# baegwangbin/MaGNet

Hardware: NVIDIA B200
Metric: frames/sec (640x480, 4 views, 64 hyp) (higher is better)
Workload: dtype f32

## Files before the change

### magnet_b200/csrc/cost_mma.cu

```cuda
#include <cuda_fp16.h>

#include <algorithm>
#include <atomic>
#include <cstddef>
#include <mutex>
#include <type_traits>

#include "common.cuh"
#include "tma_common.cuh"

namespace magnet {

constexpr int MNT = 256;
constexpr int MTW = 8, MTH = 8;
constexpr int MPX = MTW * MTH;
constexpr int MCH = 64;
constexpr int MSEG = 32;
constexpr int MMAXV = 16;
constexpr int M_TMEM_COLS = 256;
constexpr int SEG_BYTES = 2048;
constexpr int META_SEG_BYTES = 128;

constexpr int MOFF_A = 0;
constexpr int MOFF_R = 16384;
constexpr int MR_BYTES = 67584;
constexpr int MOFF_META = MOFF_R + MR_BYTES;
constexpr int MOFF_CAM = MOFF_META + MSEG * META_SEG_BYTES;
constexpr int MOFF_KS = MOFF_CAM + MMAXV * 64;
constexpr int MOFF_BBOX = MOFF_KS + MCH * 4;
constexpr int MOFF_BAR = MOFF_BBOX + 64;
constexpr int MOFF_ACC = MOFF_BAR + 64;
constexpr int MOFF_PIX = MOFF_ACC + MCH * 65 * 4;
constexpr int M_SMEM_USED = MOFF_PIX + 8 * 8 * 32;
constexpr int M_SMEM_TOTAL = M_SMEM_USED + 1024;
static_assert(MR_BYTES >= MSEG * SEG_BYTES && MR_BYTES >= MPX * 260 * 4 && MR_BYTES >= MCH * 65 * 4, "region R");
static_assert(2 * (M_SMEM_TOTAL + 1024) <= 227 * 1024, "two CTAs per SM");

struct Split16Header {
  float scale;
  float inv_scale;
  unsigned absmax;
};
constexpr size_t SPLIT16_HEADER = 256;

__host__ __device__ inline size_t split16_bytes(size_t N, size_t H, size_t W) {
  return SPLIT16_HEADER + N * H * W * 256 + N * H * (W + 1) * 16;
}

__device__ __forceinline__ void mbar_wait_or_trap(uint32_t bar, uint32_t parity) {
#pragma unroll 1
  for (int it = 0; it < (1 << 22); ++it) {
    uint32_t done;
    asm volatile("{\n.reg .pred P1;\nmbarrier.try_wait.parity.shared::cta.b64 P1, [%1], %2, %3;\nselp.u32 %0, 1, 0, P1;\n}"
                 : "=r"(done) : "r"(bar), "r"(parity), "r"(20000u) : "memory");
    if (done) return;
  }
  __trap();
}

constexpr int MMA_SLOTS = 1024;
__device__ unsigned g_mma_next[MMA_SLOTS];
__device__ unsigned g_mma_done[MMA_SLOTS];

__device__ __forceinline__ float lds_f32(uint32_t a) {
  float v;
  asm volatile("ld.shared.f32 %0, [%1];" : "=f"(v) : "r"(a));
  return v;
}
__device__ __forceinline__ float4 lds_f32x4(uint32_t a) {
  float4 v;
  asm volatile("ld.shared.v4.f32 {%0, %1, %2, %3}, [%4];" : "=f"(v.x), "=f"(v.y), "=f"(v.z), "=f"(v.w) : "r"(a));
  return v;
}
__device__ __forceinline__ float2 lerp2d_x2(float4 top, float4 bot, float fx, float fy) {
  const float2 v00 = make_float2(top.x, top.y), v01 = make_float2(top.z, top.w);
  const float2 v10 = make_float2(bot.x, bot.y), v11 = make_float2(bot.z, bot.w);
  const float2 m1 = make_float2(-1.0f, -1.0f), fx2 = make_float2(fx, fx), fy2 = make_float2(fy, fy);
  const float2 t = __ffma2_rn(fx2, __ffma2_rn(v00, m1, v01), v00), u = __ffma2_rn(fx2, __ffma2_rn(v10, m1, v11), v10);
  return __ffma2_rn(fy2, __ffma2_rn(t, m1, u), t);
}

template <int MODE, bool CW>
__global__ void __launch_bounds__(MNT, 2)
cost_mma_kernel(const __grid_constant__ CostParams p, const __grid_constant__ CUtensorMap tm_ref,
                const __grid_constant__ CUtensorMap tm_src, const __grid_constant__ CUtensorMap tm_meta, const int nchunks,
                const int n_items, const int slot, float* __restrict__ dbg) {
  extern __shared__ unsigned char smem_raw[];
  const uint32_t raw = smem_u32(smem_raw);
  const uint32_t padb = (1024u - (raw & 1023u)) & 1023u;
  unsigned char* smem = smem_raw + padb;
  const uint32_t sbase = raw + padb;
  const magnet_camera* cams_s = reinterpret_cast<const magnet_camera*>(smem + MOFF_CAM);
  float* ks = reinterpret_cast<float*>(smem + MOFF_KS);
  int* bbox = reinterpret_cast<int*>(smem + MOFF_BBOX);
  float* regR = reinterpret_cast<float*>(smem + MOFF_R);
  const uint32_t bar_tma = sbase + MOFF_BAR, bar_mma = sbase + MOFF_BAR + 8, bar_cam = sbase + MOFF_BAR + 24;
  float* acc_s = reinterpret_cast<float*>(smem + MOFF_ACC);
  const unsigned FULL = 0xffffffffu;

  const int tid = threadIdx.x, lane = tid & 31, warp = tid >> 5;
  const int H = p.H, W = p.W, HW = p.HW, D = p.D, V = p.V;
  const int tiles_x = (W + MTW - 1) / MTW;
  const int items_per_b = tiles_x * ((H + MTH - 1) / MTH) * nchunks;

  const unsigned char* refbuf = reinterpret_cast<const unsigned char*>(p.ref_feat);
  const unsigned char* srcbuf = reinterpret_cast<const unsigned char*>(p.src_feat);
  const Split16Header* hdr_ref = reinterpret_cast<const Split16Header*>(refbuf);
  const Split16Header* hdr_src = reinterpret_cast<const Split16Header*>(srcbuf);
  volatile int* next_item = reinterpret_cast<volatile int*>(smem + MOFF_BAR + 40);

  if (tid == 0) {
    mbar_init(bar_tma, 1);
    mbar_init(bar_mma, 1);
    mbar_init(bar_cam, 1);
    fence_mbar_init();
    prefetch_tmap(&tm_ref);
    prefetch_tmap(&tm_src);
    prefetch_tmap(&tm_meta);
  }
  if (warp == 1) tmem_alloc(sbase + MOFF_BAR + 32, M_TMEM_COLS);
  if (tid < 8) bbox[tid] = (tid & 1) ? -(1 << 28) : (1 << 28);
  tmem_fence_before_sync();
  __syncthreads();
  tmem_fence_after_sync();
  const uint32_t tmem_base = *reinterpret_cast<const volatile uint32_t*>(smem + MOFF_BAR + 32);
  uint32_t ph_tma = 0, ph_mma = 0, ph_cam = 0;
  int it = 0;
  int cur_b = -1;
  const float xmax = (float)W + 1.0f, ymax = (float)H + 1.0f;
  const float kappa = p.kappa;
  const uint32_t g_row0 = sbase + MOFF_R, m_base = sbase + MOFF_META;

  int item = blockIdx.x;
  while (item < n_items) {
  const int b = item / items_per_b;
  const int rem = item - b * items_per_b;
  const int tile = rem / nchunks;
  const int jc = (rem - tile * nchunks) * MCH;
  const int Dc = min(MCH, D - jc);
  const int tx0 = (tile % tiles_x) * MTW, ty0 = (tile / tiles_x) * MTH;

  if (tid == 0) {
    if (b != cur_b) {
      mbar_arrive_expect_tx(bar_cam, (uint32_t)V * 64u);
      bulk_load(sbase + MOFF_CAM, p.cams + (size_t)b * V, (uint32_t)V * 64u, bar_cam);
    }
    tma_load_5d(sbase + MOFF_A, &tm_ref, bar_tma, 0, tx0, ty0, 0, b);
    *next_item = (int)gridDim.x + (int)atomicAdd(&g_mma_next[slot], 1u);
  }
  if (tid < MCH) ks[tid] = MODE != MAGNET_DEPTH_VOLUME ? p.k[min(jc + tid, D - 1)] : 0.0f;
  for (int idx = tid; idx < MCH * 65; idx += MNT) acc_s[idx] = 0.0f;
  __syncthreads();

  const int py = ty0 + warp;
  float R0, R1, R2, MU = 0.f, SG = 0.f;
  unsigned livemask;
  {
    const int px = tx0 + (lane & 7);
    const bool live = px < W && py < H;
    const int n = min(py, H - 1) * W + min(px, W - 1);
    R0 = ldg_f(p.rays + ((size_t)b * 3 + 0) * HW + n);
    R1 = ldg_f(p.rays + ((size_t)b * 3 + 1) * HW + n);
    R2 = ldg_f(p.rays + ((size_t)b * 3 + 2) * HW + n);
    if (MODE == MAGNET_DEPTH_GAUSS) {
      MU = ldg_f(p.ref_gmm + ((size_t)b * 2 + 0) * HW + n);
      SG = ldg_f(p.ref_gmm + ((size_t)b * 2 + 1) * HW + n);
    }
    livemask = __ballot_sync(FULL, live) & 0xffu;
  }
  float2 dvol[MODE == MAGNET_DEPTH_VOLUME ? MTW : 1];
  float2 k2 = make_float2(0.f, 0.f);
  if (MODE == MAGNET_DEPTH_VOLUME) {
    for (int idx = tid; idx < MCH * MPX; idx += MNT) {
      const int j = idx >> 6, pp = idx & 63;
      const int y = ty0 + (pp >> 3), x = tx0 + (pp & 7);
      const size_t n = (size_t)min(y, H - 1) * W + min(x, W - 1);
      regR[j * 65 + pp] = ldg_f(p.d_volume + ((size_t)b * D + jc + min(j, Dc - 1)) * HW + n);
    }
    __syncthreads();
#pragma unroll
    for (int i = 0; i < MTW; ++i) dvol[i] = make_float2(regR[lane * 65 + warp * 8 + i], regR[(lane + 32) * 65 + warp * 8 + i]);
    fence_proxy_async();
    __syncthreads();
  } else {
    k2 = make_float2(ks[lane], ks[lane + 32]);
  }
  auto depth2 = [&](const int i, const float mu, const float sg) -> float2 {
    if (MODE == MAGNET_DEPTH_VOLUME) return dvol[i];
    if (MODE == MAGNET_DEPTH_PLANES) return k2;
    return __fadd2_rn(make_float2(mu, mu), make_float2(__fmul_rn(sg, k2.x), __fmul_rn(sg, k2.y)));
  };
  float4* pixt = reinterpret_cast<float4*>(smem + MOFF_PIX) + warp * 16;

  if (b != cur_b) {
    mbar_wait_or_trap(bar_cam, ph_cam);
    ph_cam ^= 1u;
    cur_b = b;
  }
  bool first = true;

  for (int v = 0; v < V; ++v) {
    const magnet_camera* cam = cams_s + v;
    if (cam->valid != 1.0f) continue;
    const float a0 = cam->a[0], a1 = cam->a[1], a2 = cam->a[2];
    const float Q0 = __fmaf_rn(cam->A[2], R2, __fmaf_rn(cam->A[1], R1, __fmul_rn(cam->A[0], R0)));
    const float Q1 = __fmaf_rn(cam->A[5], R2, __fmaf_rn(cam->A[4], R1, __fmul_rn(cam->A[3], R0)));
    const float Q2 = __fmaf_rn(cam->A[8], R2, __fmaf_rn(cam->A[7], R1, __fmul_rn(cam->A[6], R0)));
    __syncwarp();
    if (lane < 8) {
      pixt[2 * lane] = make_float4(Q0, Q1, Q2, 0.0f);
      pixt[2 * lane + 1] = make_float4(Q2, MU, SG, 0.0f);
    }
    __syncwarp();
    const int vb = v * p.B + b;

    float2 cix[MTW], ciy[MTW];
    float xl = 1e9f, xh = -1e9f, yl = 1e9f, yh = -1e9f;
#pragma unroll
    for (int i = 0; i < MTW; ++i) {
      const float4 t1 = pixt[2 * i], t2 = pixt[2 * i + 1];
      float2 ix, iy, z;
      project2(depth2(i, t2.y, t2.z), a0, a1, a2, t1.x, t1.y, t1.z, ix, iy, z);
      ix.x = fminf(fmaxf(ix.x, -2.0f), xmax); ix.y = fminf(fmaxf(ix.y, -2.0f), xmax);
      iy.x = fminf(fmaxf(iy.x, -2.0f), ymax); iy.y = fminf(fmaxf(iy.y, -2.0f), ymax);
      cix[i] = ix;
      ciy[i] = iy;
      if ((livemask >> i) & 1u) {
        xl = fminf(xl, fminf(ix.x, ix.y)); xh = fmaxf(xh, fmaxf(ix.x, ix.y));
        yl = fminf(yl, fminf(iy.x, iy.y)); yh = fmaxf(yh, fmaxf(iy.x, iy.y));
      }
    }
    int* bb = bbox + (it & 1) * 4;
    {
      const int r0 = __reduce_min_sync(FULL, (int)floorf(xl)), r1 = __reduce_max_sync(FULL, (int)floorf(xh));
      const int r2 = __reduce_min_sync(FULL, (int)floorf(yl)), r3 = __reduce_max_sync(FULL, (int)floorf(yh));
      if (lane == 0) { atomicMin(bb + 0, r0); atomicMax(bb + 1, r1); atomicMin(bb + 2, r2); atomicMax(bb + 3, r3); }
    }
    fence_proxy_async();
    __syncthreads();
    const int wx0 = bb[0], wx1 = bb[1], wy0 = bb[2], wy1 = bb[3];
    if (tid < 4) bbox[((it + 1) & 1) * 4 + tid] = (tid & 1) ? -(1 << 28) : (1 << 28);
    ++it;
    const int nseg_all = (wx1 - wx0 + 2 + 7) >> 3, rows_all = wy1 - wy0 + 2;
    const int nsw = min(nseg_all, 16);
    const int rmax = nseg_all * rows_all <= MSEG ? rows_all : max(2, MSEG / nsw);
    const int stepx = 8 * nsw - 1, stepy = rmax - 1;

    for (int sy = wy0; sy <= wy1; sy += stepy) {
      const int rows = min(stepy, wy1 - sy + 1) + 1;
      for (int sx = wx0; sx <= wx1; sx += stepx) {
        const int nseg = (min(stepx, wx1 - sx + 1) + 1 + 7) >> 3;
        const int nsegs = nseg * rows;
        if (tid == 0)
          mbar_arrive_expect_tx(bar_tma, (uint32_t)nsegs * (SEG_BYTES + (CW ? META_SEG_BYTES : 0)) + (first ? 16384u : 0u));
        first = false;
        if (lane == 0) {
          for (int s = warp; s < nsegs; s += MNT / 32) {
            const int r = s / nseg, xb = s - r * nseg;
            tma_load_5d(sbase + MOFF_R + (uint32_t)s * SEG_BYTES, &tm_src, bar_tma, 0, sx + 8 * xb, sy + r, 0, vb);
            if (CW) tma_load_4d(m_base + (uint32_t)s * META_SEG_BYTES, &tm_meta, bar_tma, 0, sx + 8 * xb + 1, sy + r, vb);
          }
        }
        __syncwarp();
        const int npad = (nsegs * 8 + 15) & ~15;
        const int gp = (((npad + 27) >> 5) << 5) + 4;
        mbar_wait_or_trap(bar_tma, ph_tma);
        ph_tma ^= 1u;
        if (warp == 0) {
          tmem_fence_after_sync();
          if (lane == 0) {
            const uint32_t idesc = umma_idesc_f16(128, (uint32_t)npad);
            const uint64_t a_hi = umma_desc_sw128(sbase + MOFF_A, 1024), a_lo = umma_desc_sw128(sbase + MOFF_A + 8192, 1024);
            const uint64_t b_hi = umma_desc_sw128(sbase + MOFF_R, SEG_BYTES), b_lo = umma_desc_sw128(sbase + MOFF_R + 1024, SEG_BYTES);
            uint32_t accum = 0;
#pragma unroll
            for (int pr = 0; pr < 3; ++pr) {
              const uint64_t ad = pr == 0 ? a_lo : a_hi, bd = pr == 1 ? b_lo : b_hi;
#pragma unroll
              for (int kk = 0; kk < 4; ++kk) {
                umma_f16(tmem_base, ad + 2u * kk, bd + 2u * kk, idesc, accum);
                accum = 1;
              }
            }
            umma_commit(bar_mma);
          }
          __syncwarp();
        }
        mbar_wait_or_trap(bar_mma, ph_mma);
        ph_mma ^= 1u;
        tmem_fence_after_sync();
        if ((warp & 3) < 2) {
          const int row = (warp & 3) * 32 + lane;
          float4* grow = reinterpret_cast<float4*>(regR + (size_t)row * gp);
          for (int cc = warp >> 2; cc * 16 < npad; cc += 2) {
            float t[16];
            tmem_ld16(tmem_base + ((uint32_t)((warp & 3) * 32) << 16) + (uint32_t)(cc * 16), t);
#pragma unroll
            for (int e = 0; e < 4; ++e) grow[cc * 4 + e] = make_float4(t[4 * e], t[4 * e + 1], t[4 * e + 2], t[4 * e + 3]);
          }
        }
        tmem_fence_before_sync();
        __syncthreads();
#ifdef MAGNET_MMA_DEBUG
        if (dbg != nullptr && item == 0 && v == 0 && sy == wy0 && sx == wx0) {
          if (tid == 0) {
            dbg[0] = (float)sx; dbg[1] = (float)sy; dbg[2] = (float)nseg; dbg[3] = (float)rows; dbg[4] = (float)npad;
            dbg[5] = (float)gp; dbg[6] = (float)v; dbg[7] = 3.0f; dbg[8] = hdr_ref->scale; dbg[9] = hdr_src->scale;
          }
          for (int idx = tid; idx < MPX * npad; idx += MNT) dbg[16 + (idx / npad) * 256 + idx % npad] = regR[(idx / npad) * gp + idx % npad];
        }
#endif
        const bool single = nseg_all * rows_all <= MSEG;
        auto phase_c = [&](auto single_tag) {
          constexpr bool SINGLE = decltype(single_tag)::value;
          const float MAGIC = 12582912.0f;
          const float sxf = (float)sx, syf = (float)sy;
          const float xend = sx + stepx > wx1 ? 1e9f : (float)(sx + stepx), yend = sy + stepy > wy1 ? 1e9f : (float)(sy + stepy);
          const float pitch4f = (float)(nseg * 32);
          const float c0f = MAGIC - 4.0f * sxf - pitch4f * syf;
          const uint32_t pitch4 = (uint32_t)nseg * 32u;
          uint32_t rowaddr = g_row0 + (uint32_t)(warp * 8 * gp) * 4u;
          float* accp = acc_s + lane * 65 + warp * 8;
#pragma unroll
          for (int i = 0; i < MTW; ++i, rowaddr += (uint32_t)gp * 4u) {
            if (!((livemask >> i) & 1u)) continue;
            asm volatile("" : "+f"(cix[i].x), "+f"(cix[i].y), "+f"(ciy[i].x), "+f"(ciy[i].y));
            const float2 x = cix[i], y = ciy[i];
            const float2 x0 = make_float2(floorf(x.x), floorf(x.y)), y0 = make_float2(floorf(y.x), floorf(y.y));
            const float2 m1 = make_float2(-1.0f, -1.0f);
            const float2 fx = __ffma2_rn(x0, m1, x), fy = __ffma2_rn(y0, m1, y);
            const float2 o = __ffma2_rn(y0, make_float2(pitch4f, pitch4f), __ffma2_rn(x0, make_float2(4.0f, 4.0f), make_float2(c0f, c0f)));
            uint32_t ca = __float_as_uint(o.x) & 0x3fffffu, cb = __float_as_uint(o.y) & 0x3fffffu;
            bool pa = true, pb = true;
            if (!SINGLE) {
              pa = x0.x >= sxf && x0.x < xend && y0.x >= syf && y0.x < yend;
              pb = x0.y >= sxf && x0.y < xend && y0.y >= syf && y0.y < yend;
              ca = pa ? ca : 0u;
              cb = pb ? cb : 0u;
            }
            const uint32_t ga = rowaddr + ca, gb = rowaddr + cb;
            const float2 g00 = make_float2(lds_f32(ga), lds_f32(gb)), g01 = make_float2(lds_f32(ga + 4), lds_f32(gb + 4));
            const float2 g10 = make_float2(lds_f32(ga + pitch4), lds_f32(gb + pitch4));
            const float2 g11 = make_float2(lds_f32(ga + pitch4 + 4), lds_f32(gb + pitch4 + 4));
            const float2 ct = __ffma2_rn(fx, __ffma2_rn(g00, m1, g01), g00), cu = __ffma2_rn(fx, __ffma2_rn(g10, m1, g11), g10);
            const float2 cost = __ffma2_rn(fy, __ffma2_rn(ct, m1, cu), ct);
            const float costa = cost.x, costb = cost.y;
            bool oka, okb;
            if (CW) {
              const uint32_t ma = m_base + ca * 4u, mb = m_base + cb * 4u;
              const float2 msa = lerp2d_x2(lds_f32x4(ma), lds_f32x4(ma + pitch4 * 4u), fx.x, fy.x);
              const float2 msb = lerp2d_x2(lds_f32x4(mb), lds_f32x4(mb + pitch4 * 4u), fx.y, fy.y);
              const float4 t2 = pixt[2 * i + 1];
              const float2 dd = depth2(i, t2.y, t2.z);
              const float2 z = __fadd2_rn(make_float2(a2, a2), make_float2(__fmul_rn(t2.x, dd.x), __fmul_rn(t2.x, dd.y)));
              oka = fabsf(__fsub_rn(z.x, msa.x)) < __fmul_rn(msa.y, kappa);
              okb = fabsf(__fsub_rn(z.y, msb.x)) < __fmul_rn(msb.y, kappa);
            } else {
              oka = fabsf(costa) < 3.0e38f;
              okb = fabsf(costb) < 3.0e38f;
            }
            if (pa && oka) accp[i] += costa;
            if (pb && okb) accp[32 * 65 + i] += costb;
          }
        };
        if (single) phase_c(std::true_type{});
        else phase_c(std::false_type{});
        fence_proxy_async();
        tmem_fence_before_sync();
        __syncthreads();
      }
    }
  }

  if (first) {
    if (tid == 0) mbar_arrive_expect_tx(bar_tma, 16384u);
    mbar_wait_or_trap(bar_tma, ph_tma);
    ph_tma ^= 1u;
  }

  {
    const float inv = hdr_ref->inv_scale * hdr_src->inv_scale;
    const bool exact = p.inv_v_exact != 0.0f;
    auto fin = [&](float a) { a *= inv; return exact ? a * p.inv_v_exact : __fdiv_rn(a, p.vf); };
    if ((W & 3) == 0 && (reinterpret_cast<uintptr_t>(p.out) & 15) == 0) {
      for (int idx = tid; idx < MCH * 16; idx += MNT) {
        const int j = idx >> 4, r = (idx >> 1) & 7, hx = (idx & 1) * 4;
        const int y = ty0 + r, x = tx0 + hx;
        if (j < Dc && x < W && y < H) {
          const float* a = acc_s + j * 65 + r * 8 + hx;
          *reinterpret_cast<float4*>(p.out + ((size_t)b * D + jc + j) * HW + (size_t)y * W + x) =
              make_float4(fin(a[0]), fin(a[1]), fin(a[2]), fin(a[3]));
        }
      }
    } else {
      for (int idx = tid; idx < MCH * MPX; idx += MNT) {
        const int j = idx >> 6, pp = idx & 63;
        const int y = ty0 + (pp >> 3), x = tx0 + (pp & 7);
        if (j < Dc && x < W && y < H) p.out[((size_t)b * D + jc + j) * HW + (size_t)y * W + x] = fin(acc_s[j * 65 + pp]);
      }
    }
  }
  const int nxt = *next_item;
  __syncthreads();
  item = nxt;
  }

  if (tid == 0) {
    __threadfence();
    if (atomicAdd(&g_mma_done[slot], 1u) == gridDim.x - 1) {
      g_mma_next[slot] = 0u;
      g_mma_done[slot] = 0u;
      __threadfence();
    }
  }
  tmem_fence_before_sync();
  __syncthreads();
  if (warp == 1) tmem_dealloc(tmem_base, M_TMEM_COLS);
}

__device__ __forceinline__ unsigned finite_abs_bits(float x) {
  const unsigned u = __float_as_uint(x) & 0x7fffffffu;
  return u >= 0x7f800000u ? 0u : u;
}

__global__ void __launch_bounds__(256) absmax_kernel(const float4* __restrict__ x, size_t n4, const float* __restrict__ tail,
                                                     int ntail, unsigned* __restrict__ out) {
  unsigned m = 0u;
  for (size_t i = (size_t)blockIdx.x * blockDim.x + threadIdx.x; i < n4; i += (size_t)gridDim.x * blockDim.x) {
    const float4 v = __ldg(x + i);
    m = max(max(m, finite_abs_bits(v.x)), finite_abs_bits(v.y));
    m = max(max(m, finite_abs_bits(v.z)), finite_abs_bits(v.w));
  }
  if (blockIdx.x == 0 && (int)threadIdx.x < ntail) m = max(m, finite_abs_bits(tail[threadIdx.x]));
  m = __reduce_max_sync(0xffffffffu, m);
  if ((threadIdx.x & 31) == 0 && m != 0u) atomicMax(out, m);
}

__device__ __forceinline__ int split16_shift(unsigned absmax_bits) {
  const int e = (int)(absmax_bits >> 23) & 0xff;
  if (e == 0 || e == 255) return 0;
  return max(-100, min(100, 14 - (e - 127)));
}

template <int SPX, bool VEC>
__global__ void __launch_bounds__(256) split16_repack_kernel(const float* __restrict__ src, const float* __restrict__ gmm,
                                                             unsigned char* __restrict__ dst, int N, int HW, int W) {
  constexpr int C = 64;
  __shared__ float t[SPX * (C + 1)];
  Split16Header* hdr = reinterpret_cast<Split16Header*>(dst);
  const int sh = split16_shift(hdr->absmax);
  const float s = __uint_as_float((unsigned)(127 + sh) << 23);
  if (blockIdx.x == 0 && blockIdx.y == 0 && threadIdx.x == 0) {
    hdr->scale = s;
    hdr->inv_scale = __uint_as_float((unsigned)(127 - sh) << 23);
  }
  const size_t img = blockIdx.y;
  const int p0 = blockIdx.x * SPX;
  if constexpr (VEC) {
    static_assert(SPX == 128, "thread mapping below");
    constexpr int CPI = 8;
    const int lane = threadIdx.x & 31, warp = threadIdx.x >> 5;
    const int q4 = (warp & 3) * 8 + (lane & 7), c0 = (warp >> 2) * 4 + (lane >> 3);
    float4 v[C / CPI];
#pragma unroll
    for (int e = 0; e < C / CPI; ++e) {
      const int c = c0 + e * CPI, pix = p0 + 4 * q4;
      v[e] = pix < HW ? __ldg(reinterpret_cast<const float4*>(src + (img * C + c) * HW + pix)) : make_float4(0.f, 0.f, 0.f, 0.f);
    }
#pragma unroll
    for (int e = 0; e < C / CPI; ++e) {
      const int c = c0 + e * CPI;
      t[(4 * q4 + 0) * (C + 1) + c] = v[e].x;
      t[(4 * q4 + 1) * (C + 1) + c] = v[e].y;
      t[(4 * q4 + 2) * (C + 1) + c] = v[e].z;
      t[(4 * q4 + 3) * (C + 1) + c] = v[e].w;
    }
  } else {
    const int xi = threadIdx.x % SPX, cy = threadIdx.x / SPX;
    for (int c = cy; c < C; c += 256 / SPX) t[xi * (C + 1) + c] = p0 + xi < HW ? src[(img * C + c) * HW + p0 + xi] : 0.0f;
  }
  __syncthreads();
  __half* planes = reinterpret_cast<__half*>(dst + SPLIT16_HEADER);
  float4* meta = reinterpret_cast<float4*>(dst + SPLIT16_HEADER + (size_t)N * HW * 256);
#pragma unroll
  for (int itw = 0; itw < SPX * 8 / 256; ++itw) {
    const int item = itw * 256 + threadIdx.x;
    const int pl = item >> 3, q = item & 7;
    if (p0 + pl < HW) {
      __align__(16) __half hi[8], lo[8];
#pragma unroll
      for (int e = 0; e < 8; ++e) {
        const float v = t[pl * (C + 1) + q * 8 + e] * s;
        hi[e] = __float2half_rn(v);
        lo[e] = __float2half_rn(v - __half2float(hi[e]));
      }
      const size_t o = (size_t)(p0 + pl) * 64 + q * 8;
      *reinterpret_cast<uint4*>(planes + (img * 2 + 0) * (size_t)HW * 64 + o) = *reinterpret_cast<const uint4*>(hi);
      *reinterpret_cast<uint4*>(planes + (img * 2 + 1) * (size_t)HW * 64 + o) = *reinterpret_cast<const uint4*>(lo);
    }
  }
  if (threadIdx.x < SPX && p0 + threadIdx.x < HW) {
    const int pix = p0 + threadIdx.x;
    const int y = pix / W, x = pix - y * W;
    float2 ms = make_float2(0.0f, 0.0f);
    if (gmm != nullptr) ms = make_float2(gmm[(img * 2 + 0) * HW + pix], gmm[(img * 2 + 1) * HW + pix]);
    float2* row = reinterpret_cast<float2*>(meta + (img * (HW / W) + y) * (size_t)(W + 1));
    row[2 * (x + 1)] = ms;
    row[2 * x + 1] = ms;
    if (x == 0) row[0] = make_float2(0.0f, 0.0f);
    if (x == W - 1) row[2 * W + 1] = make_float2(0.0f, 0.0f);
  }
}

cudaError_t launch_repack_split16(const float* src, const float* gmm, void* dst, int N, int C, int H, int W,
                                  cudaStream_t st, int* launches) {
  if (C != 64) return cudaErrorInvalidValue;
  const int HW = H * W;
  const size_t n = (size_t)N * C * HW;
  cudaError_t e = cudaMemsetAsync(dst, 0, SPLIT16_HEADER, st);
  if (e != cudaSuccess) return e;
  const size_t n4 = n / 4;
  const int blocks = (int)std::min<size_t>(148 * 8, (n4 + 255) / 256 + 1);
  absmax_kernel<<<blocks, 256, 0, st>>>(reinterpret_cast<const float4*>(src), n4, src + n4 * 4, (int)(n - n4 * 4),
                                        reinterpret_cast<unsigned*>(static_cast<unsigned char*>(dst) + offsetof(Split16Header, absmax)));
  dim3 block(256);
  if (HW % 4 == 0 && reinterpret_cast<uintptr_t>(src) % 16 == 0) {
    dim3 grid((HW + 127) / 128, N);
    split16_repack_kernel<128, true><<<grid, block, 0, st>>>(src, gmm, static_cast<unsigned char*>(dst), N, HW, W);
  } else {
    dim3 grid((HW + 31) / 32, N);
    split16_repack_kernel<32, false><<<grid, block, 0, st>>>(src, gmm, static_cast<unsigned char*>(dst), N, HW, W);
  }
  *launches = 2;
  return cudaGetLastError();
}

typedef CUresult (*EncodeTiledFn)(CUtensorMap*, CUtensorMapDataType, cuuint32_t, void*, const cuuint64_t*,
                                  const cuuint64_t*, const cuuint32_t*, const cuuint32_t*, CUtensorMapInterleave,
                                  CUtensorMapSwizzle, CUtensorMapL2promotion, CUtensorMapFloatOOBfill);
EncodeTiledFn encode_tiled_fn();

static cudaError_t make_planes_map(CUtensorMap* tm, const void* planes, int N, int H, int W, int box_rows) {
  EncodeTiledFn enc = encode_tiled_fn();
  if (!enc) return cudaErrorNotSupported;
  const cuuint64_t dims[5] = {64, (cuuint64_t)W, (cuuint64_t)H, 2, (cuuint64_t)N};
  const cuuint64_t strides[4] = {128, (cuuint64_t)W * 128, (cuuint64_t)H * W * 128, (cuuint64_t)H * W * 256};
  const cuuint32_t box[5] = {64u, 8u, (cuuint32_t)box_rows, 2u, 1u};
  const cuuint32_t estr[5] = {1u, 1u, 1u, 1u, 1u};
  const CUresult r = enc(tm, CU_TENSOR_MAP_DATA_TYPE_FLOAT16, 5, const_cast<void*>(planes), dims, strides, box, estr,
                         CU_TENSOR_MAP_INTERLEAVE_NONE, CU_TENSOR_MAP_SWIZZLE_128B, CU_TENSOR_MAP_L2_PROMOTION_L2_256B,
                         CU_TENSOR_MAP_FLOAT_OOB_FILL_NONE);
  return r == CUDA_SUCCESS ? cudaSuccess : cudaErrorInvalidValue;
}

static cudaError_t make_meta_map(CUtensorMap* tm, const void* meta, int N, int H, int W) {
  EncodeTiledFn enc = encode_tiled_fn();
  if (!enc) return cudaErrorNotSupported;
  const cuuint64_t dims[4] = {4, (cuuint64_t)W + 1, (cuuint64_t)H, (cuuint64_t)N};
  const cuuint64_t strides[3] = {16, ((cuuint64_t)W + 1) * 16, (cuuint64_t)H * (W + 1) * 16};
  const cuuint32_t box[4] = {4u, 8u, 1u, 1u};
  const cuuint32_t estr[4] = {1u, 1u, 1u, 1u};
  const CUresult r = enc(tm, CU_TENSOR_MAP_DATA_TYPE_FLOAT32, 4, const_cast<void*>(meta), dims, strides, box, estr,
                         CU_TENSOR_MAP_INTERLEAVE_NONE, CU_TENSOR_MAP_SWIZZLE_NONE, CU_TENSOR_MAP_L2_PROMOTION_L2_128B,
                         CU_TENSOR_MAP_FLOAT_OOB_FILL_NONE);
  return r == CUDA_SUCCESS ? cudaSuccess : cudaErrorInvalidValue;
}

#ifdef MAGNET_MMA_DEBUG
static float* g_mma_dbg = nullptr;
void mma_set_debug_buffer(float* p) { g_mma_dbg = p; }
#endif

static int sm_count(int dev) {
  static int cached[64] = {0};
  int& c = cached[dev & 63];
  if (c == 0) {
    int n = 0;
    if (cudaDeviceGetAttribute(&n, cudaDevAttrMultiProcessorCount, dev) != cudaSuccess || n <= 0) n = 148;
    c = n;
  }
  return c;
}

template <int MODE, bool CW>
static cudaError_t launch_mma_mw(const CostParams& p, cudaStream_t st) {
  static std::once_flag flags[64];
  auto kern = cost_mma_kernel<MODE, CW>;
  int dev = 0;
  cudaError_t e = cudaGetDevice(&dev);
  if (e != cudaSuccess) return e;
  cudaError_t res = cudaSuccess;
  std::call_once(flags[dev & 63], [&] {
    res = cudaFuncSetAttribute(kern, cudaFuncAttributeMaxDynamicSharedMemorySize, M_SMEM_TOTAL);
    if (res == cudaSuccess)
      res = cudaFuncSetAttribute(kern, cudaFuncAttributePreferredSharedMemoryCarveout, cudaSharedmemCarveoutMaxShared);
  });
  if (res != cudaSuccess) return res;
  const int N = p.B * p.V;
  const unsigned char* refbuf = reinterpret_cast<const unsigned char*>(p.ref_feat);
  const unsigned char* srcbuf = reinterpret_cast<const unsigned char*>(p.src_feat);
  CUtensorMap tm_ref, tm_src, tm_meta;
  if ((e = make_planes_map(&tm_ref, refbuf + SPLIT16_HEADER, p.B, p.H, p.W, 8)) != cudaSuccess) return e;
  if ((e = make_planes_map(&tm_src, srcbuf + SPLIT16_HEADER, N, p.H, p.W, 1)) != cudaSuccess) return e;
  if ((e = make_meta_map(&tm_meta, srcbuf + SPLIT16_HEADER + (size_t)N * p.HW * 256, N, p.H, p.W)) != cudaSuccess) return e;
  const int nchunks = (p.D + MCH - 1) / MCH;
  const int tiles = ((p.W + MTW - 1) / MTW) * ((p.H + MTH - 1) / MTH);
  const int n_items = tiles * nchunks * p.B;
  static std::atomic<unsigned> ticket{0}, graph_ticket{0};
  cudaStreamCaptureStatus cap = cudaStreamCaptureStatusNone;
  if (cudaStreamIsCapturing(st, &cap) != cudaSuccess) cap = cudaStreamCaptureStatusNone;
  const int slot = cap == cudaStreamCaptureStatusActive ? MMA_SLOTS / 2 + (int)(graph_ticket.fetch_add(1) % (MMA_SLOTS / 2))
                                                        : (int)(ticket.fetch_add(1) % (MMA_SLOTS / 2));
  dim3 grid(std::min(n_items, 2 * sm_count(dev))), block(MNT);
  float* dbg = nullptr;
#ifdef MAGNET_MMA_DEBUG
  dbg = g_mma_dbg;
#endif
  kern<<<grid, block, M_SMEM_TOTAL, st>>>(p, tm_ref, tm_src, tm_meta, nchunks, n_items, slot, dbg);
  return cudaGetLastError();
}

bool mma_supports(int C, int D, int V, int layout) {
  return C == 64 && layout == MAGNET_SRC_SPLIT16 && D >= 1 && V <= MMAXV;
}

void mma_launch_info(int B, int H, int W, int D, int* grid, int* block, int* smem) {
  int dev = 0;
  cudaGetDevice(&dev);
  *grid = std::min(((W + MTW - 1) / MTW) * ((H + MTH - 1) / MTH) * ((D + MCH - 1) / MCH) * B, 2 * sm_count(dev));
  *block = MNT;
  *smem = M_SMEM_TOTAL;
}

size_t split16_buffer_bytes(int N, int H, int W) { return split16_bytes((size_t)N, (size_t)H, (size_t)W); }

cudaError_t launch_cost_mma(const CostParams& p, int mode, bool cw, cudaStream_t st) {
  if (cw) {
    if (mode == MAGNET_DEPTH_VOLUME) return launch_mma_mw<MAGNET_DEPTH_VOLUME, true>(p, st);
    if (mode == MAGNET_DEPTH_GAUSS) return launch_mma_mw<MAGNET_DEPTH_GAUSS, true>(p, st);
    return launch_mma_mw<MAGNET_DEPTH_PLANES, true>(p, st);
  }
  if (mode == MAGNET_DEPTH_VOLUME) return launch_mma_mw<MAGNET_DEPTH_VOLUME, false>(p, st);
  if (mode == MAGNET_DEPTH_GAUSS) return launch_mma_mw<MAGNET_DEPTH_GAUSS, false>(p, st);
  return launch_mma_mw<MAGNET_DEPTH_PLANES, false>(p, st);
}

}
```

Before: 9386.

## Precompute per-view bounding boxes and keep accumulators in registers

```diff
diff --git a/magnet_b200/csrc/cost_mma.cu b/magnet_b200/csrc/cost_mma.cu
--- a/magnet_b200/csrc/cost_mma.cu
+++ b/magnet_b200/csrc/cost_mma.cu
@@ -27,13 +27,13 @@
 constexpr int MOFF_META = MOFF_R + MR_BYTES;
 constexpr int MOFF_CAM = MOFF_META + MSEG * META_SEG_BYTES;
 constexpr int MOFF_KS = MOFF_CAM + MMAXV * 64;
-constexpr int MOFF_BBOX = MOFF_KS + MCH * 4;
-constexpr int MOFF_BAR = MOFF_BBOX + 64;
-constexpr int MOFF_ACC = MOFF_BAR + 64;
-constexpr int MOFF_PIX = MOFF_ACC + MCH * 65 * 4;
+constexpr int MOFF_BOX = MOFF_KS + MCH * 4;
+constexpr int MOFF_BAR = MOFF_BOX + MMAXV * 20;
+constexpr int MOFF_PIX = MOFF_BAR + 64;
 constexpr int M_SMEM_USED = MOFF_PIX + 8 * 8 * 32;
 constexpr int M_SMEM_TOTAL = M_SMEM_USED + 1024;
 static_assert(MR_BYTES >= MSEG * SEG_BYTES && MR_BYTES >= MPX * 260 * 4 && MR_BYTES >= MCH * 65 * 4, "region R");
+static_assert(MOFF_BAR % 8 == 0 && MOFF_PIX % 16 == 0, "mbarrier / float4 alignment");
 static_assert(2 * (M_SMEM_TOTAL + 1024) <= 227 * 1024, "two CTAs per SM");
 
 struct Split16Header {
@@ -78,6 +78,24 @@
   const float2 m1 = make_float2(-1.0f, -1.0f), fx2 = make_float2(fx, fx), fy2 = make_float2(fy, fy);
   const float2 t = __ffma2_rn(fx2, __ffma2_rn(v00, m1, v01), v00), u = __ffma2_rn(fx2, __ffma2_rn(v10, m1, v11), v10);
   return __ffma2_rn(fy2, __ffma2_rn(t, m1, u), t);
+}
+
+__device__ __forceinline__ bool extreme_box(float dlo, float dhi, float a0, float a1, float a2, float q0, float q1,
+                                            float q2, float xmax, float ymax, int& bx0, int& bx1, int& by0, int& by1) {
+  float2 ix, iy, z;
+  project2(make_float2(dlo, dhi), a0, a1, a2, q0, q1, q2, ix, iy, z);
+  const float zmin = fminf(fabsf(z.x), fabsf(z.y));
+  const float top = fabsf(a2) + fmaxf(fabsf(__fmul_rn(q2, dlo)), fabsf(__fmul_rn(q2, dhi)));
+  const float xm = fmaxf(fmaxf(fabsf(ix.x), fabsf(ix.y)), fmaxf(fabsf(iy.x), fabsf(iy.y)));
+  const bool finite = fabsf(ix.x) <= 1e30f && fabsf(ix.y) <= 1e30f && fabsf(iy.x) <= 1e30f && fabsf(iy.y) <= 1e30f &&
+                      fabsf(z.x) <= 1e30f && fabsf(z.y) <= 1e30f;
+  const bool ok = finite && (z.x > 0.0f) == (z.y > 0.0f) && zmin >= 1e-6f && top <= 1024.0f * zmin;
+  const float eps = (xm + 1.0f) * (8.0f + top / zmin) * 0x1p-22f;
+  bx0 = (int)floorf(fminf(fmaxf(fminf(ix.x, ix.y) - eps, -2.0f), xmax));
+  bx1 = (int)floorf(fminf(fmaxf(fmaxf(ix.x, ix.y) + eps, -2.0f), xmax));
+  by0 = (int)floorf(fminf(fmaxf(fminf(iy.x, iy.y) - eps, -2.0f), ymax));
+  by1 = (int)floorf(fminf(fmaxf(fmaxf(iy.x, iy.y) + eps, -2.0f), ymax));
+  return ok;
 }
 
 template <int MODE, bool CW>
@@ -92,10 +110,10 @@
   const uint32_t sbase = raw + padb;
   const magnet_camera* cams_s = reinterpret_cast<const magnet_camera*>(smem + MOFF_CAM);
   float* ks = reinterpret_cast<float*>(smem + MOFF_KS);
-  int* bbox = reinterpret_cast<int*>(smem + MOFF_BBOX);
+  int* vbox = reinterpret_cast<int*>(smem + MOFF_BOX);
+  int* vexact = vbox + MMAXV * 4;
   float* regR = reinterpret_cast<float*>(smem + MOFF_R);
   const uint32_t bar_tma = sbase + MOFF_BAR, bar_mma = sbase + MOFF_BAR + 8, bar_cam = sbase + MOFF_BAR + 24;
-  float* acc_s = reinterpret_cast<float*>(smem + MOFF_ACC);
   const unsigned FULL = 0xffffffffu;
 
   const int tid = threadIdx.x, lane = tid & 31, warp = tid >> 5;
@@ -119,13 +137,11 @@
     prefetch_tmap(&tm_meta);
   }
   if (warp == 1) tmem_alloc(sbase + MOFF_BAR + 32, M_TMEM_COLS);
-  if (tid < 8) bbox[tid] = (tid & 1) ? -(1 << 28) : (1 << 28);
   tmem_fence_before_sync();
   __syncthreads();
   tmem_fence_after_sync();
   const uint32_t tmem_base = *reinterpret_cast<const volatile uint32_t*>(smem + MOFF_BAR + 32);
   uint32_t ph_tma = 0, ph_mma = 0, ph_cam = 0;
-  int it = 0;
   int cur_b = -1;
   const float xmax = (float)W + 1.0f, ymax = (float)H + 1.0f;
   const float kappa = p.kappa;
@@ -149,7 +165,8 @@
     *next_item = (int)gridDim.x + (int)atomicAdd(&g_mma_next[slot], 1u);
   }
   if (tid < MCH) ks[tid] = MODE != MAGNET_DEPTH_VOLUME ? p.k[min(jc + tid, D - 1)] : 0.0f;
-  for (int idx = tid; idx < MCH * 65; idx += MNT) acc_s[idx] = 0.0f;
+  if (tid < MMAXV * 4) vbox[tid] = (tid & 1) ? -(1 << 28) : (1 << 28);
+  if (tid < MMAXV) vexact[tid] = MODE != MAGNET_DEPTH_VOLUME && !p.k_sorted;
   __syncthreads();
 
   const int py = ty0 + warp;
@@ -170,6 +187,8 @@
   }
   float2 dvol[MODE == MAGNET_DEPTH_VOLUME ? MTW : 1];
   float2 k2 = make_float2(0.f, 0.f);
+  float dlo, dhi;
+  bool dbad;
   if (MODE == MAGNET_DEPTH_VOLUME) {
     for (int idx = tid; idx < MCH * MPX; idx += MNT) {
       const int j = idx >> 6, pp = idx & 63;
@@ -182,65 +201,118 @@
     for (int i = 0; i < MTW; ++i) dvol[i] = make_float2(regR[lane * 65 + warp * 8 + i], regR[(lane + 32) * 65 + warp * 8 + i]);
     fence_proxy_async();
     __syncthreads();
+    unsigned nonfinite = 0u;
+    dlo = 0.0f; dhi = 0.0f;
+#pragma unroll
+    for (int i = 0; i < MTW; ++i) {
+      float lo = fminf(dvol[i].x, dvol[i].y), hi = fmaxf(dvol[i].x, dvol[i].y);
+      if (!(isfinite(dvol[i].x) && isfinite(dvol[i].y))) nonfinite |= 1u << i;
+#pragma unroll
+      for (int o = 16; o > 0; o >>= 1) {
+        lo = fminf(lo, __shfl_xor_sync(FULL, lo, o));
+        hi = fmaxf(hi, __shfl_xor_sync(FULL, hi, o));
+      }
+      if ((lane & 7) == i) { dlo = lo; dhi = hi; }
+    }
+    dbad = (__reduce_or_sync(FULL, nonfinite) >> (lane & 7)) & 1u;
   } else {
     k2 = make_float2(ks[lane], ks[lane + 32]);
-  }
+    const float k0 = ks[0], k1 = ks[Dc - 1];
+    const float e0 = MODE == MAGNET_DEPTH_PLANES ? k0 : __fadd_rn(MU, __fmul_rn(SG, k0));
+    const float e1 = MODE == MAGNET_DEPTH_PLANES ? k1 : __fadd_rn(MU, __fmul_rn(SG, k1));
+    dlo = fminf(e0, e1);
+    dhi = fmaxf(e0, e1);
+    dbad = !(isfinite(e0) && isfinite(e1));
+  }
+  auto kray = [&](const magnet_camera* cam) -> float3 {
+    return make_float3(__fmaf_rn(cam->A[2], R2, __fmaf_rn(cam->A[1], R1, __fmul_rn(cam->A[0], R0))),
+                       __fmaf_rn(cam->A[5], R2, __fmaf_rn(cam->A[4], R1, __fmul_rn(cam->A[3], R0))),
+                       __fmaf_rn(cam->A[8], R2, __fmaf_rn(cam->A[7], R1, __fmul_rn(cam->A[6], R0))));
+  };
   auto depth2 = [&](const int i, const float mu, const float sg) -> float2 {
     if (MODE == MAGNET_DEPTH_VOLUME) return dvol[i];
     if (MODE == MAGNET_DEPTH_PLANES) return k2;
     return __fadd2_rn(make_float2(mu, mu), make_float2(__fmul_rn(sg, k2.x), __fmul_rn(sg, k2.y)));
   };
   float4* pixt = reinterpret_cast<float4*>(smem + MOFF_PIX) + warp * 16;
+  if (lane < 8) pixt[2 * lane + 1] = make_float4(MU, SG, 0.0f, 0.0f);
 
   if (b != cur_b) {
     mbar_wait_or_trap(bar_cam, ph_cam);
     ph_cam ^= 1u;
     cur_b = b;
   }
+
+  for (int v0 = 0; v0 < V; v0 += 4) {
+    const int v = v0 + (lane >> 3);
+    const magnet_camera* cam = cams_s + min(v, V - 1);
+    const float3 Q = kray(cam);
+    int r0, r1, r2, r3;
+    bool ok = extreme_box(dlo, dhi, cam->a[0], cam->a[1], cam->a[2], Q.x, Q.y, Q.z, xmax, ymax, r0, r1, r2, r3) && !dbad;
+    const bool counts = v < V && cam->valid == 1.0f && ((livemask >> (lane & 7)) & 1u);
+    if (!counts) ok = true;
+    if (!(counts && ok)) { r0 = 1 << 28; r1 = -(1 << 28); r2 = 1 << 28; r3 = -(1 << 28); }
+#pragma unroll
+    for (int o = 1; o < 8; o <<= 1) {
+      r0 = min(r0, __shfl_xor_sync(FULL, r0, o)); r1 = max(r1, __shfl_xor_sync(FULL, r1, o));
+      r2 = min(r2, __shfl_xor_sync(FULL, r2, o)); r3 = max(r3, __shfl_xor_sync(FULL, r3, o));
+    }
+    const bool fails = (__ballot_sync(FULL, !ok) >> (lane & 24)) & 0xffu;
+    if ((lane & 7) == 0 && v < V) {
+      atomicMin(vbox + 4 * v + 0, r0); atomicMax(vbox + 4 * v + 1, r1);
+      atomicMin(vbox + 4 * v + 2, r2); atomicMax(vbox + 4 * v + 3, r3);
+      if (fails) vexact[v] = 1;
+    }
+  }
+  __syncthreads();
+  {
+    bool any = false;
+    for (int v = 0; v < V; ++v) {
+      const magnet_camera* cam = cams_s + v;
+      if (!vexact[v] || cam->valid != 1.0f) continue;
+      any = true;
+      const float3 Q = kray(cam);
+      float xl = 1e9f, xh = -1e9f, yl = 1e9f, yh = -1e9f;
+#pragma unroll
+      for (int i = 0; i < MTW; ++i) {
+        const float q0 = __shfl_sync(FULL, Q.x, i), q1 = __shfl_sync(FULL, Q.y, i), q2 = __shfl_sync(FULL, Q.z, i);
+        const float mu = __shfl_sync(FULL, MU, i), sg = __shfl_sync(FULL, SG, i);
+        float2 ix, iy, z;
+        project2(depth2(i, mu, sg), cam->a[0], cam->a[1], cam->a[2], q0, q1, q2, ix, iy, z);
+        ix.x = fminf(fmaxf(ix.x, -2.0f), xmax); ix.y = fminf(fmaxf(ix.y, -2.0f), xmax);
+        iy.x = fminf(fmaxf(iy.x, -2.0f), ymax); iy.y = fminf(fmaxf(iy.y, -2.0f), ymax);
+        if ((livemask >> i) & 1u) {
+          xl = fminf(xl, fminf(ix.x, ix.y)); xh = fmaxf(xh, fmaxf(ix.x, ix.y));
+          yl = fminf(yl, fminf(iy.x, iy.y)); yh = fmaxf(yh, fmaxf(iy.x, iy.y));
+        }
+      }
+      const int r0 = __reduce_min_sync(FULL, (int)floorf(xl)), r1 = __reduce_max_sync(FULL, (int)floorf(xh));
+      const int r2 = __reduce_min_sync(FULL, (int)floorf(yl)), r3 = __reduce_max_sync(FULL, (int)floorf(yh));
+      if (lane == 0) {
+        atomicMin(vbox + 4 * v + 0, r0); atomicMax(vbox + 4 * v + 1, r1);
+        atomicMin(vbox + 4 * v + 2, r2); atomicMax(vbox + 4 * v + 3, r3);
+      }
+    }
+    if (any) __syncthreads();
+  }
+
+  float2 acc[MTW];
+#pragma unroll
+  for (int i = 0; i < MTW; ++i) acc[i] = make_float2(0.0f, 0.0f);
   bool first = true;
 
   for (int v = 0; v < V; ++v) {
     const magnet_camera* cam = cams_s + v;
     if (cam->valid != 1.0f) continue;
     const float a0 = cam->a[0], a1 = cam->a[1], a2 = cam->a[2];
-    const float Q0 = __fmaf_rn(cam->A[2], R2, __fmaf_rn(cam->A[1], R1, __fmul_rn(cam->A[0], R0)));
-    const float Q1 = __fmaf_rn(cam->A[5], R2, __fmaf_rn(cam->A[4], R1, __fmul_rn(cam->A[3], R0)));
-    const float Q2 = __fmaf_rn(cam->A[8], R2, __fmaf_rn(cam->A[7], R1, __fmul_rn(cam->A[6], R0)));
-    __syncwarp();
-    if (lane < 8) {
-      pixt[2 * lane] = make_float4(Q0, Q1, Q2, 0.0f);
-      pixt[2 * lane + 1] = make_float4(Q2, MU, SG, 0.0f);
-    }
-    __syncwarp();
+    {
+      const float3 Q = kray(cam);
+      __syncwarp();
+      if (lane < 8) pixt[2 * lane] = make_float4(Q.x, Q.y, Q.z, 0.0f);
+      __syncwarp();
+    }
     const int vb = v * p.B + b;
-
-    float2 cix[MTW], ciy[MTW];
-    float xl = 1e9f, xh = -1e9f, yl = 1e9f, yh = -1e9f;
-#pragma unroll
-    for (int i = 0; i < MTW; ++i) {
-      const float4 t1 = pixt[2 * i], t2 = pixt[2 * i + 1];
-      float2 ix, iy, z;
-      project2(depth2(i, t2.y, t2.z), a0, a1, a2, t1.x, t1.y, t1.z, ix, iy, z);
-      ix.x = fminf(fmaxf(ix.x, -2.0f), xmax); ix.y = fminf(fmaxf(ix.y, -2.0f), xmax);
-      iy.x = fminf(fmaxf(iy.x, -2.0f), ymax); iy.y = fminf(fmaxf(iy.y, -2.0f), ymax);
-      cix[i] = ix;
-      ciy[i] = iy;
-      if ((livemask >> i) & 1u) {
-        xl = fminf(xl, fminf(ix.x, ix.y)); xh = fmaxf(xh, fmaxf(ix.x, ix.y));
-        yl = fminf(yl, fminf(iy.x, iy.y)); yh = fmaxf(yh, fmaxf(iy.x, iy.y));
-      }
-    }
-    int* bb = bbox + (it & 1) * 4;
-    {
-      const int r0 = __reduce_min_sync(FULL, (int)floorf(xl)), r1 = __reduce_max_sync(FULL, (int)floorf(xh));
-      const int r2 = __reduce_min_sync(FULL, (int)floorf(yl)), r3 = __reduce_max_sync(FULL, (int)floorf(yh));
-      if (lane == 0) { atomicMin(bb + 0, r0); atomicMax(bb + 1, r1); atomicMin(bb + 2, r2); atomicMax(bb + 3, r3); }
-    }
-    fence_proxy_async();
-    __syncthreads();
-    const int wx0 = bb[0], wx1 = bb[1], wy0 = bb[2], wy1 = bb[3];
-    if (tid < 4) bbox[((it + 1) & 1) * 4 + tid] = (tid & 1) ? -(1 << 28) : (1 << 28);
-    ++it;
+    const int wx0 = vbox[4 * v + 0], wx1 = vbox[4 * v + 1], wy0 = vbox[4 * v + 2], wy1 = vbox[4 * v + 3];
     const int nseg_all = (wx1 - wx0 + 2 + 7) >> 3, rows_all = wy1 - wy0 + 2;
     const int nsw = min(nseg_all, 16);
     const int rmax = nseg_all * rows_all <= MSEG ? rows_all : max(2, MSEG / nsw);
@@ -319,18 +391,28 @@
           const float pitch4f = (float)(nseg * 32);
           const float c0f = MAGIC - 4.0f * sxf - pitch4f * syf;
           const uint32_t pitch4 = (uint32_t)nseg * 32u;
+          const uint32_t maxoff = pitch4 * (uint32_t)(rows - 2) + 4u * (uint32_t)(8 * nseg - 2);
           uint32_t rowaddr = g_row0 + (uint32_t)(warp * 8 * gp) * 4u;
-          float* accp = acc_s + lane * 65 + warp * 8;
 #pragma unroll
           for (int i = 0; i < MTW; ++i, rowaddr += (uint32_t)gp * 4u) {
             if (!((livemask >> i) & 1u)) continue;
-            asm volatile("" : "+f"(cix[i].x), "+f"(cix[i].y), "+f"(ciy[i].x), "+f"(ciy[i].y));
-            const float2 x = cix[i], y = ciy[i];
+            const float4 t1 = pixt[2 * i];
+            float2 d;
+            if (MODE == MAGNET_DEPTH_GAUSS) {
+              const float4 t2 = pixt[2 * i + 1];
+              d = depth2(i, t2.x, t2.y);
+            } else {
+              d = depth2(i, 0.0f, 0.0f);
+            }
+            float2 x, y, z;
+            project2(d, a0, a1, a2, t1.x, t1.y, t1.z, x, y, z);
+            x.x = fminf(fmaxf(x.x, -2.0f), xmax); x.y = fminf(fmaxf(x.y, -2.0f), xmax);
+            y.x = fminf(fmaxf(y.x, -2.0f), ymax); y.y = fminf(fmaxf(y.y, -2.0f), ymax);
             const float2 x0 = make_float2(floorf(x.x), floorf(x.y)), y0 = make_float2(floorf(y.x), floorf(y.y));
             const float2 m1 = make_float2(-1.0f, -1.0f);
             const float2 fx = __ffma2_rn(x0, m1, x), fy = __ffma2_rn(y0, m1, y);
             const float2 o = __ffma2_rn(y0, make_float2(pitch4f, pitch4f), __ffma2_rn(x0, make_float2(4.0f, 4.0f), make_float2(c0f, c0f)));
-            uint32_t ca = __float_as_uint(o.x) & 0x3fffffu, cb = __float_as_uint(o.y) & 0x3fffffu;
+            uint32_t ca = min(__float_as_uint(o.x) & 0x3fffffu, maxoff), cb = min(__float_as_uint(o.y) & 0x3fffffu, maxoff);
             bool pa = true, pb = true;
             if (!SINGLE) {
               pa = x0.x >= sxf && x0.x < xend && y0.x >= syf && y0.x < yend;
@@ -350,17 +432,14 @@
               const uint32_t ma = m_base + ca * 4u, mb = m_base + cb * 4u;
               const float2 msa = lerp2d_x2(lds_f32x4(ma), lds_f32x4(ma + pitch4 * 4u), fx.x, fy.x);
               const float2 msb = lerp2d_x2(lds_f32x4(mb), lds_f32x4(mb + pitch4 * 4u), fx.y, fy.y);
-              const float4 t2 = pixt[2 * i + 1];
-              const float2 dd = depth2(i, t2.y, t2.z);
-              const float2 z = __fadd2_rn(make_float2(a2, a2), make_float2(__fmul_rn(t2.x, dd.x), __fmul_rn(t2.x, dd.y)));
               oka = fabsf(__fsub_rn(z.x, msa.x)) < __fmul_rn(msa.y, kappa);
               okb = fabsf(__fsub_rn(z.y, msb.x)) < __fmul_rn(msb.y, kappa);
             } else {
               oka = fabsf(costa) < 3.0e38f;
               okb = fabsf(costb) < 3.0e38f;
             }
-            if (pa && oka) accp[i] += costa;
-            if (pb && okb) accp[32 * 65 + i] += costb;
+            if (pa && oka) acc[i].x += costa;
+            if (pb && okb) acc[i].y += costb;
           }
         };
         if (single) phase_c(std::true_type{});
@@ -383,21 +462,32 @@
     const bool exact = p.inv_v_exact != 0.0f;
     auto fin = [&](float a) { a *= inv; return exact ? a * p.inv_v_exact : __fdiv_rn(a, p.vf); };
     if ((W & 3) == 0 && (reinterpret_cast<uintptr_t>(p.out) & 15) == 0) {
-      for (int idx = tid; idx < MCH * 16; idx += MNT) {
-        const int j = idx >> 4, r = (idx >> 1) & 7, hx = (idx & 1) * 4;
-        const int y = ty0 + r, x = tx0 + hx;
-        if (j < Dc && x < W && y < H) {
-          const float* a = acc_s + j * 65 + r * 8 + hx;
-          *reinterpret_cast<float4*>(p.out + ((size_t)b * D + jc + j) * HW + (size_t)y * W + x) =
-              make_float4(fin(a[0]), fin(a[1]), fin(a[2]), fin(a[3]));
+      if (py < H) {
+        float* o = p.out + ((size_t)b * D + jc + lane) * HW + (size_t)py * W + tx0;
+        const bool full = tx0 + 4 < W;
+        if (lane < Dc) {
+          reinterpret_cast<float4*>(o)[0] = make_float4(fin(acc[0].x), fin(acc[1].x), fin(acc[2].x), fin(acc[3].x));
+          if (full) reinterpret_cast<float4*>(o)[1] = make_float4(fin(acc[4].x), fin(acc[5].x), fin(acc[6].x), fin(acc[7].x));
+        }
+        if (lane + 32 < Dc) {
+          o += (size_t)32 * HW;
+          reinterpret_cast<float4*>(o)[0] = make_float4(fin(acc[0].y), fin(acc[1].y), fin(acc[2].y), fin(acc[3].y));
+          if (full) reinterpret_cast<float4*>(o)[1] = make_float4(fin(acc[4].y), fin(acc[5].y), fin(acc[6].y), fin(acc[7].y));
         }
       }
     } else {
+#pragma unroll
+      for (int i = 0; i < MTW; ++i) {
+        regR[lane * 65 + warp * 8 + i] = acc[i].x;
+        regR[(lane + 32) * 65 + warp * 8 + i] = acc[i].y;
+      }
+      __syncthreads();
       for (int idx = tid; idx < MCH * MPX; idx += MNT) {
         const int j = idx >> 6, pp = idx & 63;
         const int y = ty0 + (pp >> 3), x = tx0 + (pp & 7);
-        if (j < Dc && x < W && y < H) p.out[((size_t)b * D + jc + j) * HW + (size_t)y * W + x] = fin(acc_s[j * 65 + pp]);
+        if (j < Dc && x < W && y < H) p.out[((size_t)b * D + jc + j) * HW + (size_t)y * W + x] = fin(regR[j * 65 + pp]);
       }
+      fence_proxy_async();
     }
   }
   const int nxt = *next_item;
```

Result: faster. 9580 (median of 6 runs) (+2.1%).
